# ducha-aiki/mods

Measured on AMD Instinct MI355X. Metric: image-pairs/sec (1024x768, HessAff+RootSIFT over the affine view ladder, MFMA FGINN match, LO-RANSAC H), higher is better.
Workload: dtype f32 (detect/describe) + u8 on the int8 matrix cores (distance matrix)

## Files before the change

### mods_amd/csrc/engine.hpp

```cpp
#pragma once
#include <hip/hip_runtime.h>
#include <stdint.h>
#include <stdlib.h>
#include <string.h>
#include <string>
#include <vector>
#include "../../include/modsx.h"
#include "kmath.hpp"

namespace mx {

#ifndef MODSX_MAXB
#define MODSX_MAXB 32
#endif
constexpr int MAXB = MODSX_MAXB;
constexpr int PAIR_GROUP = 4;
constexpr int NMS_MAXJ = 1024;
constexpr int MAX_TAPS = 17;

struct BlurJob {
  const float *src;
  float *blur;
  float *resp;
  int rows, cols;
// ... 8 lines not shown
  int tile0[MAXB + 1];
};
struct ResizeJob {
  const float *src;
  float *dst;
  float *resp;
  int srows, scols, drows, dcols;
  float norm;
  int pad;
};
struct ResizeBatch { ResizeJob j[MAXB]; int nj; int tile0[MAXB + 1]; };
struct NmsJob {
  const float *low, *cur, *high, *blur;
  int rows, cols, img, octave, level, pad;
};
struct NmsBatch {
  float posTh, negTh, finalTh;
  int border;
  double edgeScoreThreshold;
  int detType, pad;
};
struct Candidate {
  int img, octave, level, type;
  int r0, c0, r, c;
  float b0, b1, b2, val;
};

struct AffJob {
  const float *blur;
  int rows, cols;
  float x, y, s, pixelDistance;
};
struct AffOut { float u11, u12, u21, u22; int ok; int iters; };

struct OriJob {
  int img;
  float x, y, a11, a12, a21, a22;
};
constexpr int ORI_MAX_PEAKS = 18;

struct DescJob {
  int img;
  int P;
  int ksize;
  int tapOfs;
  float x, y, a11, a12, a21, a22;
  float i2p;
  int NC;
  int needOfs;
  int coordOfs;
  int touch;
  int outIdx;
  int rows0;
  int ro1;
  unsigned long long scratchOfs;
  unsigned long long rowOfs;
  unsigned long long gridOfs;
};
struct BlurTile {
  unsigned long long srcOfs, dstOfs;
  int P, NC, n, tapOfs, needOfs;
  int job, pad;
  int first, count, lo, span, magic;
};
struct ImgRef { const float *d; int rows, cols, pad; };
struct DescOut { float *f[MAXB]; uint8_t *u8[MAXB]; uint8_t *u8x[3][MAXB]; };

struct WarpJob {
  const float *src;
  float *dst;
  int srows, scols, drows, dcols;
  double M[6];
  float cval;
  int pad;
};

struct ViewJob {
  const float *src;
  float *rot, *tmp, *dst;
  int srows, scols, rrows, rcols, drows, dcols;
  int kx, ky, tapOfs, doBlur;
  int tileA, tileB;
  int tileF, fused;
  double R[6], W[6];
};

struct MatchRow {
  int t0, t1, nless, nbad;
  int tj;
  float dj;
  float d0, d1;
};
static_assert(sizeof(MatchRow) == 32, "match rows are 32 bytes");

struct DevBuf {
  void *p = nullptr;
  size_t cap = 0;
  bool ensure(size_t bytes);
  void release();
};
struct PinBuf {
  void *p = nullptr;
  size_t cap = 0;
  bool ensure(size_t bytes);
  void release();
};

struct Octave {
  int rows, cols;
  float pixelDistance;
  float *blur[8];
  float *resp[8];
};
struct Pyramid {
  int nOct = 0;
  Octave oct[24];
  DevBuf store;
};

void set_error(const std::string &s);
bool gpu_shared();
struct CtxBusy { modsx_ctx *c; explicit CtxBusy(modsx_ctx *c); ~CtxBusy(); CtxBusy(const CtxBusy &) = delete; CtxBusy &operator=(const CtxBusy &) = delete; };
hipError_t ctx_copy(modsx_ctx *c, void *dst, const void *src, size_t bytes, hipMemcpyKind kind);
hipError_t ctx_sync(modsx_ctx *c);
unsigned ctx_mark(modsx_ctx *c);
bool ctx_mark_reached(modsx_ctx *c, unsigned seq);
hipError_t ctx_wait_mark(modsx_ctx *c, unsigned seq);
bool host_wait_runtime();
int host_cpus_per_rank();
#define MX_HIP(expr)                                                                          \
  do {                                                                                        \
    hipError_t e_ = (expr);                                                                   \
    if (e_ != hipSuccess) {                                                                   \
      mx::set_error(std::string(#expr) + ": " + hipGetErrorString(e_));                       \
      return MODSX_ERR_DEVICE;                                                                \
    }                                                                                         \
  } while (0)

std::vector<float> gaussian_kernel(int n, double sigma);
int blur_ksize(float sigma);
void gauss_mask(float *mask, int size);
void circular_gauss_mask(float *mask, int size, float sigma);
const double *atan_lut_host();
inline bool check_borders_host(int w, int h, float ofsx, float ofsy, float a11, float a12, float a21, float a22, int rw, int rh) {
  return check_borders(w, h, ofsx, ofsy, a11, a12, a21, a22, rw, rh);
}
bool invert3(const double *S, double *t);
void rectify(double &a11, double &a12, double &a21, double &a22);

void launch_blur_hess(hipStream_t s, const BlurBatch &b, int nj, int maxRows, int maxCols);
void launch_hessian(hipStream_t s, const BlurBatch &b, int nj, int maxRows, int maxCols);
void launch_resize_half(hipStream_t s, const ResizeBatch &b, int nj, int maxRows, int maxCols);
void launch_nms(hipStream_t s, const NmsBatch &b, const NmsJob *jobs, const int *tilePrefix, const int *tileJob, int nj,
                int nTiles, int4 *queue, unsigned *qcount, unsigned qcap, Candidate *out, unsigned *counter, unsigned cap,
                const int *octFirst = nullptr, int levelsPerOctave = 0);
size_t cand_sort_temp_bytes(unsigned nsort);
int launch_cand_order(hipStream_t s, const Candidate *cand, const unsigned *counter, unsigned nsort, unsigned long long *keys,
                      unsigned long long *keys2, unsigned *idx, unsigned *idx2, void *temp, size_t tempBytes, unsigned long long *tabKey,
                      unsigned *tabRank, unsigned tabSize, unsigned *slotOf, Candidate *out, unsigned *outCount);
constexpr int NMS_QUEUES = 64;
constexpr int NMS_TILE_ROWS = 16;
void launch_gray(hipStream_t s, const void *src, float *dst, size_t n, int channels, int dtype);
void launch_baumberg(hipStream_t s, const AffJob *jobs, AffOut *out, int n, const float *mask, int W, int maxIter,
                     float convTh, float affInitialSigma);
constexpr int ATAN_CASES = 2048 + 64;
constexpr int ORI_NV = 1344;
void launch_orientation(hipStream_t s, const OriJob *jobs, float *out, int n, const ImgRef *imgs,
                        const unsigned short *maskIdx, const float *maskW,
                        const unsigned char *binTab, int doHalf, double th, int maxAngles);
void launch_trunc_u8(hipStream_t s, const float *src, uint8_t *dst, size_t n);
size_t mser_sort_blocks(const int *rows, int n);
void launch_mser_sort(hipStream_t s, const uint8_t *const *u8, const int *rows, const int *cols, const size_t *ordOfs, int n, int *blockHist,
                      int *start, int *order);
void launch_expand_blur_tiles(hipStream_t s, const DescJob *jobs, const int *prefixRows, const int *prefixCols, int nJobs,
                              const int *needTab, BlurTile *tilesRows, BlurTile *tilesCols, float2 *rowStarts);
void launch_sample_rows(hipStream_t s, const DescJob *jobs, const BlurTile *tiles, int nTiles, const ImgRef *imgs, const float *taps,
                        const int *needTab, float *dst, const float2 *rowStarts, float *dstGrid);
void launch_blur_cols(hipStream_t s, const BlurTile *tiles, int nTiles, const float *taps, const int *needTab, const float *src,
                      float *dst);
void launch_expand_tiles(hipStream_t s, const int *prefix, int nJobs, int *tileJob);
void launch_patch_sample(hipStream_t s, const DescJob *jobs, const int *tilePrefix, const int *tileJob, int nTiles,
                         const ImgRef *imgs, float *scratch);
void launch_patch_blur(hipStream_t s, const DescJob *jobs, const int *tilePrefix, const int *tileJob, int nTiles,
                       const float *taps, const int *needTab, const float *src, float *dst, int pass);
void launch_describe(hipStream_t s, const DescJob *jobs, int n, const ImgRef *imgs, const float *grid,
                     const int *needTab, const float *coordTab,
                     const float *mask, const unsigned short *maskIdx, int nmask, const float *oTab, const int *bins,
                     const double *wts, int photoNorm, int descTypes, int nOut, double maxBin, const DescOut &outs);
void launch_warp_affine(hipStream_t s, const WarpJob &jb);
void launch_blur_pass(hipStream_t s, const float *src, float *dst, int rows, int cols, const float *taps, int n, int pass, int border = 0);
void launch_sub(hipStream_t s, const float *a, const float *b, float *o, size_t n);
void launch_grad_products(hipStream_t s, const float *img, int rows, int cols, float *xx, float *yy, float *xy);
void launch_harris_combine(hipStream_t s, const float *bxx, const float *byy, const float *bxy, float sigmasq, float *o, size_t n);
void launch_views_warp(hipStream_t s, const ViewJob *jobs, int n, int tiles, int stage);
void launch_views_blur(hipStream_t s, const ViewJob *jobs, int n, int tiles, const float *taps, int pass);
constexpr int VF_TW = 128, VF_TH = 16, VF_RX = 32, VF_RY = 2;
void launch_views_rotblur(hipStream_t s, const ViewJob *jobs, int n, int tiles, const float *taps, int maxRx, int maxRy);
size_t match_workspace_bytes(int n1, int n2);
void launch_match(hipStream_t s, const uint8_t *d1, int n1, const uint8_t *d2, int n2, const double *pos2,
                  double sqminratio, double contrDistSq, int nn, MatchRow *rows, void *workspace);
#ifndef MODSX_SR_WIN
#define MODSX_SR_WIN 2400
#define MODSX_FC_ROWS 40
#define MODSX_SR_HALF 1
#define MODSX_SR_WGS 8
#endif
#ifndef MODSX_BLUR_LDS_C
#define MODSX_BLUR_LDS_C 9984
#endif
constexpr int MATCH_NN_MAX = 256;
constexpr int MATCH_MAXB = 4;
void launch_match_batch(hipStream_t s, int nb, const uint8_t *const *d1, const int *n1, const uint8_t *const *d2, const int *n2,
                        const double *const *pos2, double sqminratio, double contrDistSq, int nn, MatchRow *const *rows,
                        void *const *workspace, hipEvent_t *evSweep1 = nullptr);

}

namespace mx {
#ifdef MODSX_DUP_BUILD
int dup_count(int cls);
#define MX_DUP(cls) for (int dupLeft_ = mx::dup_count(cls); dupLeft_ > 0; dupLeft_--)
#else
#define MX_DUP(cls)
#endif
enum KClass { K_BLUR_HESS = 0, K_HESSIAN, K_RESIZE, K_NMS, K_BAUMBERG, K_ORIENT, K_PATCH_SAMPLE, K_BLUR_ROWS, K_DESCRIBE,
              K_MATCH, K_GRAY, K_WARP, K_VIEW_BLUR, K_BLUR_COLS, K_MATCH_SWEEP1, K_NCLASS };
struct Profiler {
  bool enabled = false;
  std::vector<hipEvent_t> evA, evB;
  std::vector<int> cls;
  size_t used = 0;
  double ms[K_NCLASS] = {0};
  double work[K_NCLASS] = {0};
  long launches[K_NCLASS] = {0};
};
}

struct modsx_image {
  float *d;
  int rows, cols;
  bool owned;
};

struct modsx_ctx {
  int dev;
  hipStream_t stream;
  mx::Pyramid pyr[mx::MAXB];
  mx::DevBuf candSort, candOut;
  size_t lastSurvivors = 0;
  mx::DevBuf nmsJobs, cand, counter, affJobs, affOut, oriJobs, oriOut, descJobs, tilePrefix, taps, imgRefs, scratchA, scratchB,
      descF[mx::MAXB], descU8[mx::MAXB], descAllF[2], descAllU8[2], descAllU8b[2], descCls[2][4][2], descU8x[3][mx::MAXB], shardLocal, pos2, matchRows, matchWork, misc, viewTmp[2], viewTaps, viewJobs, viewImg[mx::MAXB], scratchC, needTab, coordTab, tileJob, blurTiles, nmsQueue, rowStarts;
  mx::ImgRef imgRefsHost[mx::MAXB];
  mx::PinBuf hDescB;
  hipEvent_t descEv[2];
  bool descEvPending[2] = {false, false};
  bool descByEvent[2] = {true, true};
  unsigned descMark[2] = {0, 0};
  unsigned *hFlag = nullptr;
  unsigned flagSeq = 0;
  bool waitRuntime = true;
  mx::PinBuf hCand, hAff, hOri, hDesc, hMisc, hNms, hMatch, hViewTaps, hViewJobs, hMser, hRefs;
  float *dSmmMask = nullptr;
  int smmW = 0;
  std::vector<uint64_t> candKeys, candKeys2, candClaim;
  std::vector<uint32_t> candOrder, candOrder2;
  float *dOriMask = nullptr;
  unsigned short *dOriIdx = nullptr;
  float *dSiftMask = nullptr;
  unsigned short *dSiftMaskIdx = nullptr;
  int nSiftMask = 0;
  double *dAtan = nullptr;
  unsigned char *dOriBinTab = nullptr;
  float *dSiftOTab = nullptr;
  int *dSiftBins = nullptr;
  double *dSiftW = nullptr;
  double timings[6];
  mx::Profiler prof;
  size_t lastCandCount = 0;
  int busyDepth = 0;
  int shardLane = 0;
// ... 6 lines not shown
```

### mods_amd/csrc/engine_views.hip

```cpp
#include <math.h>
#include <algorithm>
#include <atomic>
#include <condition_variable>
#include <functional>
#include <mutex>
#include <thread>
#include "engine_api.hpp"

namespace mx {

int set_vs_pars(const double *scale_set, int ns, const double *tilt_set, int nt, double phi_base, double InitSigma,
                int doBlur, modsx_view *par, int cap, modsx_view *prev, int *nprev, int cap_prev) {
  const double eps1 = 0.01;
  std::vector<modsx_view> tmp;
  auto mk = [&](double phi, double tilt, double zoom, int blur) {
    modsx_view v; v.phi = phi; v.tilt = tilt; v.zoom = zoom; v.InitSigma = InitSigma; v.doBlur = blur;
    return v;
  };
  if (ns == 0 || nt == 0) tmp.push_back(mk(0, 0, 0, 0));
  for (int sc = 0; sc < ns; sc++)
    for (int t = 0; t < nt; t++) {
      if (fabs(tilt_set[t] - 1) > eps1) {
        int n_rot1 = floor(180.0 * tilt_set[t] / phi_base);
        double delta_phi = M_PI / n_rot1;
// ... 54 lines not shown
    P.ow = w; P.oh = h;
    return MODSX_OK;
  }
  P.identity = 0;
  double d, d2, w_new, h_new;
  double kV = 1., kH = 1.;
  if (zoomed) { kV = (double)w / (double)wS1; kH = (double)h / (double)hS1; }
  const bool q1 = (phi >= 0) && (phi < M_PI / 2);
  if (vertical_tilt) {
    if (q1) {
      w_new = floor((0.5 + cos(phi) * w + sin(phi) * h) / (kH));
      h_new = floor((0.5 + sin(phi) * w + cos(phi) * h) / (tilt * kV));
      H[0] = cos(phi) / kH; H[1] = sin(phi) / kH; H[2] = 0;
      H[3] = -sin(phi) / (tilt * kV); H[4] = cos(phi) / (tilt * kV); H[5] = floor(0.5 + sin(phi) * w / (tilt * kV));
    } else {
      w_new = floor((0.5 - cos(phi) * w + sin(phi) * h) / (kH));
      h_new = floor((0.5 + sin(phi) * w - cos(phi) * h) / (tilt * kV));
      d = -floor(cos(phi) * w / kH);
      d2 = floor(0.5 + (sin(phi) * w - cos(phi) * h) / (tilt * kV));
      H[0] = cos(phi) / kH; H[1] = sin(phi) / kH; H[2] = d;
      H[3] = -sin(phi) / (tilt * kV); H[4] = cos(phi) / (tilt * kV); H[5] = d2;
    }
  } else {
    if (q1) {
      w_new = floor((0.5 + cos(phi) * w + sin(phi) * h) / (tilt * kH));
      h_new = floor((0.5 + sin(phi) * w + cos(phi) * h) / (kV));
      H[0] = cos(phi) / (tilt * kH); H[1] = sin(phi) / (tilt * kH); H[2] = 0;
      H[3] = -sin(phi) / kV; H[4] = cos(phi) / kV; H[5] = floor(0.5 + sin(phi) * w / kV);
    } else {
      w_new = floor((0.5 - cos(phi) * w + sin(phi) * h) / (tilt * kH));
      h_new = floor((0.5 + sin(phi) * w - cos(phi) * h) / (kV));
      d = -floor(cos(phi) * w / (tilt * kH));
      d2 = floor(0.5 + (sin(phi) * w - cos(phi) * h) / kV);
      H[0] = cos(phi) / (tilt * kH); H[1] = sin(phi) / (tilt * kH); H[2] = d;
      H[3] = -sin(phi) / kV; H[4] = cos(phi) / kV; H[5] = d2;
    }
  }
  H[6] = 0; H[7] = 0; H[8] = 1;
  double sigma_aa_2 = zoomed ? InitSigma / (4.0 * zoom) : InitSigma / 2.0;
  double sigma_aa = InitSigma * tilt / (2.0 * zoom);
  double sigma_x = vertical_tilt ? sigma_aa_2 : sigma_aa, sigma_y = vertical_tilt ? sigma_aa : sigma_aa_2;
  double R[6];
  if (q1) {
    P.w_rot = floor((0.5 + cos(phi) * w + sin(phi) * h));
    P.h_rot = floor((0.5 + sin(phi) * w + cos(phi) * h));
    R[0] = cos(phi); R[1] = sin(phi); R[2] = 0;
    R[3] = -sin(phi); R[4] = cos(phi); R[5] = floor(0.5 + sin(phi) * w);
  } else {
    P.w_rot = floor((0.5 - cos(phi) * w + sin(phi) * h));
    P.h_rot = floor((0.5 + sin(phi) * w - cos(phi) * h));
    d = -floor(cos(phi) * w);
    d2 = floor(0.5 + (sin(phi) * w - cos(phi) * h));
    R[0] = cos(phi); R[1] = sin(phi); R[2] = d;
    R[3] = -sin(phi); R[4] = cos(phi); R[5] = d2;
  }
  P.ow = (int)w_new; P.oh = (int)h_new;
  if (P.w_rot <= 0 || P.h_rot <= 0 || P.ow <= 0 || P.oh <= 0) { set_error("degenerate synthesised view"); return MODSX_ERR_ARG; }
  invert_affine(R, P.Rinv);
  P.doBlur = v.doBlur;
  P.taps.clear();
  if (v.doBlur) {
    int kx = floor(2.0 * 3.0 * sigma_x + 1.0);
    if (kx % 2 == 0) kx++;
    if (kx < 3) kx = 3;
    int ky = floor(2.0 * 3.0 * sigma_y + 1.0);
    if (ky % 2 == 0) ky++;
    if (ky < 3) ky = 3;
    if (P.h_rot == 1) ky = 1;
    if (P.w_rot == 1) kx = 1;
    std::vector<float> KX = gaussian_kernel(kx, std::max(sigma_x, 0.));
    std::vector<float> KY = (ky == kx && fabs(sigma_x - sigma_y) < 2.220446049250313e-16) ? KX : gaussian_kernel(ky, std::max(sigma_y, 0.));
    P.kx = kx; P.ky = ky;
    P.taps = KX;
    P.taps.insert(P.taps.end(), KY.begin(), KY.end());
  }
  double Wz[6] = {0, 0, 0, 0, 0, 0};
  if (vertical_tilt) { Wz[0] = 1.0 / kH; Wz[4] = 1.0 / (tilt * kV); }
  else { Wz[0] = 1.0 / (tilt * kH); Wz[4] = 1.0 / kV; }
  invert_affine(Wz, P.Winv);
  return MODSX_OK;
}

static int synth_views_batch(modsx_ctx *c, const modsx_image *const *grays, const ViewPlan *P, float *const *dst, int n) {
  hipStream_t s = c->stream;
  std::vector<ViewJob> jobs;
  std::vector<float> taps;
  size_t rotFloats = 0;
  int tilesA = 0, tilesB = 0, tilesF = 0, maxRx = 0, maxRy = 0;
  double wpx = 0, rpx = 0;
  for (int i = 0; i < n; i++) {
    if (P[i].identity) continue;
    ViewJob j;
    memset(&j, 0, sizeof j);
    const modsx_image *gray = grays[i];
    j.src = gray->d; j.srows = gray->rows; j.scols = gray->cols;
    j.rrows = P[i].h_rot; j.rcols = P[i].w_rot; j.drows = P[i].oh; j.dcols = P[i].ow;
    j.dst = dst[i];
    j.doBlur = P[i].doBlur; j.kx = P[i].kx; j.ky = P[i].ky; j.tapOfs = (int)taps.size();
    taps.insert(taps.end(), P[i].taps.begin(), P[i].taps.end());
    for (int q = 0; q < 6; q++) { j.R[q] = P[i].Rinv[q]; j.W[q] = P[i].Winv[q]; }
    j.tileA = tilesA; j.tileB = tilesB; j.tileF = tilesF;
    j.fused = j.doBlur && (j.kx >> 1) <= VF_RX && (j.ky >> 1) <= VF_RY;
    if (j.fused) {
      tilesF += ((j.rcols + VF_TW - 1) / VF_TW) * ((j.rrows + VF_TH - 1) / VF_TH);
      maxRx = std::max(maxRx, j.kx >> 1); maxRy = std::max(maxRy, j.ky >> 1);
    } else
      tilesA += ((j.rcols + 63) / 64) * ((j.rrows + 3) / 4);
    tilesB += ((j.dcols + 63) / 64) * ((j.drows + 3) / 4);
    j.rot = (float *)(uintptr_t)rotFloats;
    rotFloats += (size_t)j.rrows * j.rcols;
    wpx += (double)gray->rows * gray->cols + 2.0 * j.rrows * j.rcols + (double)j.drows * j.dcols;
    rpx += (double)j.rrows * j.rcols;
    jobs.push_back(j);
  }
  if (jobs.empty()) return MODSX_OK;
  const size_t jobB = jobs.size() * sizeof(ViewJob), tapB = std::max<size_t>(1, taps.size()) * 4;
  if (!c->viewTmp[0].ensure(rotFloats * 4) || !c->viewTmp[1].ensure(rotFloats * 4) || !c->viewJobs.ensure(jobB + tapB + 64) ||
      !c->hViewJobs.ensure(jobB + tapB + 64))
    return MODSX_ERR_NOMEM;
  for (ViewJob &j : jobs) {
    const size_t o = (size_t)(uintptr_t)j.rot;
    j.rot = (float *)c->viewTmp[0].p + o;
    j.tmp = (float *)c->viewTmp[1].p + o;
  }
  char *hb = (char *)c->hViewJobs.p;
  memcpy(hb, jobs.data(), jobB);
  if (!taps.empty()) memcpy(hb + jobB, taps.data(), taps.size() * 4);
  MX_HIP(ctx_copy(c, c->viewJobs.p, hb, jobB + tapB, hipMemcpyHostToDevice));
  const ViewJob *dj = (const ViewJob *)c->viewJobs.p;
  const float *dt = (const float *)((char *)c->viewJobs.p + jobB);
  size_t pslot;
  prof_begin(c, K_WARP, wpx * 4, &pslot);
  launch_views_warp(s, dj, (int)jobs.size(), tilesA, 0);
  prof_end(c, pslot);
  prof_begin(c, K_VIEW_BLUR, rpx * 16, &pslot);
  launch_views_rotblur(s, dj, (int)jobs.size(), tilesF, dt, maxRx, maxRy);
  launch_views_blur(s, dj, (int)jobs.size(), tilesA, dt, 0);
  launch_views_blur(s, dj, (int)jobs.size(), tilesA, dt, 1);
  prof_end(c, pslot);
  prof_begin(c, K_WARP, 0, &pslot);
  launch_views_warp(s, dj, (int)jobs.size(), tilesB, 1);
  prof_end(c, pslot);
  MX_HIP(hipGetLastError());
  return MODSX_OK;
}

int synth_view(modsx_ctx *c, const modsx_image *gray, const modsx_view &v, modsx_image **out, double *H, int *identity, int) {
  *out = nullptr;
  ViewPlan P;
  int rc = plan_view(gray, v, P);
  if (rc) return rc;
  for (int i = 0; i < 9; i++) H[i] = P.H[i];
  *identity = P.identity;
  modsx_image *im = new modsx_image();
  im->rows = P.oh; im->cols = P.ow;
  if (P.identity) { im->d = gray->d; im->owned = false; *out = im; return MODSX_OK; }
  im->owned = true; im->d = nullptr;
  if (hipMalloc(&im->d, (size_t)P.ow * P.oh * 4) != hipSuccess) { delete im; set_error("hipMalloc view"); return MODSX_ERR_NOMEM; }
  float *dst[1] = {im->d};
  rc = synth_views_batch(c, &gray, &P, dst, 1);
  if (!rc && ctx_sync(c) != hipSuccess) { set_error("view synthesis failed"); rc = MODSX_ERR_DEVICE; }
  if (rc) { hipFree(im->d); delete im; return rc; }
  *out = im;
  return MODSX_OK;
}

int detect_describe_items(modsx_ctx *c, const modsx_image *const *itemImg, const int *itemView, int nitems, const modsx_view *views,
                          const modsx_pair_params &pp, std::vector<modsx_region> &regs,
                          float *devF, uint8_t *devU8, size_t devCapRegions, float *hostDesc, int *itemCounts,
                          const DescSet *dsIn, uint8_t *const *devU8x) {
  CtxBusy busy(c);
  regs.clear();
  DescSet ds;
  if (dsIn) ds = *dsIn;
  else { const int rd = resolve_descs(pp, nullptr, ds); if (rd) return rd; }
  const int oriHalf = ds.half() ? 1 : 0;
  if (!devU8x) { ds.forceHalf = oriHalf != 0; ds.n = 1; }
  if (itemCounts) for (int k = 0; k < nitems; k++) itemCounts[k] = 0;
  struct SetScope { SetScope() { host_set_enter(); } ~SetScope() { host_set_leave(); } } setScope;
  std::vector<int> take(nitems);
  for (int k = 0; k < nitems; k++) take[k] = k;
  size_t total = 0;
  for (size_t g0 = 0; g0 < take.size(); g0 += MAXB) {
    const int n = (int)std::min<size_t>(MAXB, take.size() - g0);
    modsx_image *vimg[MAXB];
    const modsx_image *cimg[MAXB];
    double Hs[MAXB][9], tilts[MAXB], zooms[MAXB];
    int ident[MAXB];
    int rc = MODSX_OK;
    for (int i = 0; i < n; i++) vimg[i] = nullptr;
    ViewPlan plans[MAXB];
    float *vdst[MAXB];
    const modsx_image *gimg[MAXB];
    for (int i = 0; i < n && !rc; i++) {
      const modsx_image *gray = itemImg[take[g0 + i]];
      gimg[i] = gray;
      const modsx_view &v = views[itemView[take[g0 + i]]];
      rc = plan_view(gray, v, plans[i]);
      if (rc) break;
      for (int q = 0; q < 9; q++) Hs[i][q] = plans[i].H[q];
      ident[i] = plans[i].identity;
      modsx_image *im = new modsx_image();
      im->rows = plans[i].oh; im->cols = plans[i].ow; im->owned = false;
      if (ident[i]) im->d = gray->d;
      else if (!c->viewImg[i].ensure((size_t)im->rows * im->cols * 4)) { delete im; rc = MODSX_ERR_NOMEM; break; }
      else im->d = (float *)c->viewImg[i].p;
      vdst[i] = im->d;
      vimg[i] = im;
      cimg[i] = im;
      tilts[i] = ident[i] ? 1.0 : fabs(v.tilt);
      zooms[i] = ident[i] ? 1.0 : v.zoom;
    }
    auto tnow = []() { return std::chrono::duration<double, std::milli>(std::chrono::steady_clock::now().time_since_epoch()).count(); };
    const bool tim = getenv("MODSX_HOST_TIMING") != nullptr;
    const bool tim2 = tim && atoi(getenv("MODSX_HOST_TIMING")) >= 2;
    double tq = 0;
    double t0 = tnow();
    if (!rc) rc = synth_views_batch(c, gimg, plans, vdst, n);
    if (tim) hipStreamSynchronize(c->stream);
    double t1 = tnow();
    std::vector<modsx_keypoint> kps[MAXB];
    std::vector<modsx_region> r0[MAXB], ro[MAXB];
    if (!rc) {
      if (pp.detector == MODSX_DET_MSER) {
        static const bool devSort = !(getenv("MODSX_MSER_DEVICE_SORT") && !atoi(getenv("MODSX_MSER_DEVICE_SORT")));
// ... 467 lines not shown
```

### mods_amd/csrc/kernels_views.hip

```cpp
#include "engine.hpp"

namespace mx {

MX_D void warp_xterm(const double *M, int x, int &adelta, int &bdelta) {
  const int AB_SCALE = 1024;
  adelta = (int)rint(M[0] * x * AB_SCALE); bdelta = (int)rint(M[3] * x * AB_SCALE);
}
MX_D void warp_yterm(const double *M, int y, int &X0, int &Y0) {
  const int AB_SCALE = 1024;
  X0 = (int)rint((M[1] * y + M[2]) * AB_SCALE) + 16;
  Y0 = (int)rint((M[4] * y + M[5]) * AB_SCALE) + 16;
}
MX_D float warp_fetch(const float *src, int sh, int sw, float cval, int adelta, int bdelta, int X0, int Y0) {
  const int X = (X0 + adelta) >> 5, Y = (Y0 + bdelta) >> 5;
  int sx = X >> 5, sy = Y >> 5;
  sx = sx < -32768 ? -32768 : (sx > 32767 ? 32767 : sx);
  sy = sy < -32768 ? -32768 : (sy > 32767 ? 32767 : sy);
  const float fx = (float)(X & 31) * (1.f / 32), fy = (float)(Y & 31) * (1.f / 32);
  const float w0 = (1.f - fy) * (1.f - fx), w1 = (1.f - fy) * fx, w2 = fy * (1.f - fx), w3 = fy * fx;
  float out;
  if (sx >= 0 && sx < sw - 1 && sy >= 0 && sy < sh - 1) {
    const float *S = src + (size_t)sy * sw + sx;
    out = S[0] * w0 + S[1] * w1 + S[sw] * w2 + S[sw + 1] * w3;
  } else if (sx >= sw || sx + 1 < 0 || sy >= sh || sy + 1 < 0) {
    out = cval;
  } else {
    const bool x0 = sx >= 0 && sx < sw, x1 = sx + 1 >= 0 && sx + 1 < sw, y0 = sy >= 0 && sy < sh, y1 = sy + 1 >= 0 && sy + 1 < sh;
    const float v0 = (x0 && y0) ? src[(size_t)sy * sw + sx] : cval;
    const float v1 = (x1 && y0) ? src[(size_t)sy * sw + sx + 1] : cval;
    const float v2 = (x0 && y1) ? src[(size_t)(sy + 1) * sw + sx] : cval;
    const float v3 = (x1 && y1) ? src[(size_t)(sy + 1) * sw + sx + 1] : cval;
    out = v0 * w0 + v1 * w1 + v2 * w2 + v3 * w3;
  }
  return out;
}
MX_D float warp_value(const float *src, int sh, int sw, const double *M, float cval, int x, int y) {
  int ad, bd, X0, Y0;
  warp_xterm(M, x, ad, bd);
  warp_yterm(M, y, X0, Y0);
  return warp_fetch(src, sh, sw, cval, ad, bd, X0, Y0);
}
MX_D void warp_body(const WarpJob &jb, int x, int y) {
  if (x >= jb.dcols || y >= jb.drows) return;
  jb.dst[(size_t)y * jb.dcols + x] = warp_value(jb.src, jb.srows, jb.scols, jb.M, jb.cval, x, y);
}
__global__ __launch_bounds__(256) void k_warp_affine(WarpJob jb) {
  warp_body(jb, blockIdx.x * 64 + (threadIdx.x & 63), blockIdx.y * 4 + (threadIdx.x >> 6));
}

MX_D int reflect101(int p, int n) {
  if (n == 1) return 0;
  while (p < 0 || p >= n) { if (p < 0) p = -p; else p = 2 * n - 2 - p; }
  return p;
}

MX_D int border_idx(int p, int n, int border) {
  if (border) return p < 0 ? 0 : (p > n - 1 ? n - 1 : p);
  return reflect101(p, n);
}
MX_D void blur_body(const float *src, float *dst, int rows, int cols, const float *taps, int n, int pass, int x, int y, int border = 0) {
  if (x >= cols || y >= rows) return;
  const int R = n >> 1;
  float v;
  if (n == 1) v = src[(size_t)y * cols + x];
  else if (pass == 0) {
    const float *row = src + (size_t)y * cols;
    if (n <= 5) {
      v = row[x] * taps[R];
      for (int j = 1; j <= R; j++) v = v + (row[border_idx(x - j, cols, border)] + row[border_idx(x + j, cols, border)]) * taps[R + j];
    } else {
      v = 0.f;
      for (int j = 0; j < n; j++) v = v + row[border_idx(x + j - R, cols, border)] * taps[j];
    }
  } else {
    v = taps[R] * src[(size_t)y * cols + x] + 0.f;
    for (int j = 1; j <= R; j++)
      v = v + taps[R + j] * (src[(size_t)border_idx(y + j, rows, border) * cols + x] + src[(size_t)border_idx(y - j, rows, border) * cols + x]);
  }
  dst[(size_t)y * cols + x] = v;
}
__global__ __launch_bounds__(256) void k_blur_pass(const float *src, float *dst, int rows, int cols, const float *taps,
                                                   int n, int pass, int border) {
  blur_body(src, dst, rows, cols, taps, n, pass, blockIdx.x * 64 + (threadIdx.x & 63), blockIdx.y * 4 + (threadIdx.x >> 6), border);
}

__global__ __launch_bounds__(256) void k_sub(const float *a, const float *b, float *o, size_t n) {
  const size_t i = (size_t)blockIdx.x * 256 + threadIdx.x;
  if (i < n) o[i] = a[i] - b[i];
}
__global__ __launch_bounds__(256) void k_grad_products(const float *img, int rows, int cols, float *xx, float *yy, float *xy) {
  const int c = blockIdx.x * 64 + (threadIdx.x & 63), r = blockIdx.y * 4 + (threadIdx.x >> 6);
  if (c >= cols || r >= rows) return;
  const float *R = img + (size_t)r * cols;
  float xg, yg;
  if (cols == 1) xg = 0.f;
  else if (c == 0) xg = R[c + 1] - R[c];
  else if (c == cols - 1) xg = R[c] - R[c - 1];
  else xg = R[c + 1] - R[c - 1];
  if (rows == 1) yg = 0.f;
  else if (r == 0) yg = R[cols + c] - R[c];
  else if (r == rows - 1) yg = R[c] - R[c - cols];
  else yg = R[cols + c] - R[c - cols];
  const size_t i = (size_t)r * cols + c;
  xx[i] = xg * xg; yy[i] = yg * yg; xy[i] = xg * yg;
}
__global__ __launch_bounds__(256) void k_harris_combine(const float *bxx, const float *byy, const float *bxy, float sigmasq, float *o, size_t n) {
  const size_t i = (size_t)blockIdx.x * 256 + threadIdx.x;
  if (i >= n) return;
  const float dx2 = bxx[i] * sigmasq, dy2 = byy[i] * sigmasq, dxdy = bxy[i] * sigmasq;
  const float s = dx2 + dy2;
  const float a = dx2 * dy2, b = dxdy * dxdy, c = (0.04f * s) * s;
  o[i] = (a - b) - c;
}

MX_D int find_view(const ViewJob *jobs, int n, int tile, int stage) {
  int j = 0;
  while (j + 1 < n && tile >= (stage == 2 ? jobs[j + 1].tileF : (stage ? jobs[j + 1].tileB : jobs[j + 1].tileA))) j++;
  return j;
}
__global__ __launch_bounds__(256) void k_views_warp(const ViewJob *jobs, int n, int stage) {
  const int j = find_view(jobs, n, blockIdx.x, stage);
  const ViewJob &v = jobs[j];
  WarpJob jb;
  if (stage == 0) { jb.src = v.src; jb.dst = v.rot; jb.srows = v.srows; jb.scols = v.scols; jb.drows = v.rrows; jb.dcols = v.rcols; }
  else { jb.src = v.rot; jb.dst = v.dst; jb.srows = v.rrows; jb.scols = v.rcols; jb.drows = v.drows; jb.dcols = v.dcols; }
#pragma unroll
  for (int i = 0; i < 6; i++) jb.M[i] = stage ? v.W[i] : v.R[i];
  jb.cval = 128.f;
  const int t = blockIdx.x - (stage ? v.tileB : v.tileA), tx = (jb.dcols + 63) / 64;
  warp_body(jb, (t % tx) * 64 + (threadIdx.x & 63), (t / tx) * 4 + (threadIdx.x >> 6));
}
__global__ __launch_bounds__(256) void k_views_blur(const ViewJob *jobs, int n, const float *taps, int pass) {
  const int j = find_view(jobs, n, blockIdx.x, 0);
  const ViewJob &v = jobs[j];
  if (!v.doBlur) return;
  const int t = blockIdx.x - v.tileA, tx = (v.rcols + 63) / 64;
  const float *src = pass ? v.tmp : v.rot;
  float *dst = pass ? v.rot : v.tmp;
  blur_body(src, dst, v.rrows, v.rcols, taps + v.tapOfs + (pass ? v.kx : 0), pass ? v.ky : v.kx, pass, (t % tx) * 64 + (threadIdx.x & 63),
            (t / tx) * 4 + (threadIdx.x >> 6));
}

template <int N>
MX_D void vf_rows(const float *Wt, float *Tt, const float *kxT, int WW, int Rx, int lane, int ty, int xOut, int yEnd, int nxRt) {
  constexpr int NK = N ? N : 1;
  float k[NK];
#pragma unroll
  for (int q = 0; q < NK; q++) k[q] = N ? kxT[q] : 0.f;
  for (int ly = ty; ly < yEnd; ly += 4) {
    const float *row = Wt + ly * WW + Rx;
    for (int lx = lane; lx < xOut; lx += 64) {
      float r;
      if (N == 1) r = row[lx];
      else if (N == 3 || N == 5) {
        constexpr int R = N >> 1;
        r = row[lx] * k[R];
#pragma unroll
        for (int q = 1; q <= R; q++) r = r + (row[lx - q] + row[lx + q]) * k[R + q];
      } else if (N > 5) {
        constexpr int R = N >> 1;
        r = 0.f;
#pragma unroll
        for (int q = 0; q < N; q++) r = r + row[lx + q - R] * k[q];
      } else {
        const int nx = nxRt;
        if (nx <= 5) {
          r = row[lx] * kxT[Rx];
          for (int q = 1; q <= Rx; q++) r = r + (row[lx - q] + row[lx + q]) * kxT[Rx + q];
        } else {
          r = 0.f;
          for (int q = 0; q < nx; q++) r = r + row[lx + q - Rx] * kxT[q];
        }
      }
      Tt[ly * VF_TW + lx] = r;
    }
  }
}
template <int N>
MX_D void vf_cols(const float *Tt, float *outBase, const float *kyT, int rcols, int Ry, int lane, int ty, int xOut, int yOut, int nyRt) {
  constexpr int NK = N ? N : 1;
  float k[NK];
#pragma unroll
  for (int q = 0; q < NK; q++) k[q] = N ? kyT[q] : 0.f;
  for (int ly = ty; ly < yOut; ly += 4) {
    const float *col = Tt + (ly + Ry) * VF_TW;
    float *out = outBase + (size_t)ly * rcols;
    for (int lx = lane; lx < xOut; lx += 64) {
      float r;
      if (N == 1) r = col[lx];
      else if (N > 1) {
        constexpr int R = N >> 1;
        r = k[R] * col[lx] + 0.f;
#pragma unroll
        for (int q = 1; q <= R; q++) r = r + k[R + q] * (col[lx + q * VF_TW] + col[lx - q * VF_TW]);
      } else {
        (void)nyRt;
        r = kyT[Ry] * col[lx] + 0.f;
        for (int q = 1; q <= Ry; q++) r = r + kyT[Ry + q] * (col[lx + q * VF_TW] + col[lx - q * VF_TW]);
      }
      out[lx] = r;
    }
  }
}

__global__ __launch_bounds__(256) void k_views_rotblur(const ViewJob *jobs, int n, const float *taps, int wFloats) {
  extern __shared__ float smem[];
  const int j = find_view(jobs, n, blockIdx.x, 2);
  const ViewJob &v = jobs[j];
  const int Rx = v.kx >> 1, Ry = v.ky >> 1;
  const int t = blockIdx.x - v.tileF, tx = (v.rcols + VF_TW - 1) / VF_TW;
  const int x0 = (t % tx) * VF_TW, y0 = (t / tx) * VF_TH;
  const int WW = VF_TW + 2 * Rx;
  float *const Wt = smem, *const Tt = smem + wFloats;
  const int lane = threadIdx.x & 63, ty = threadIdx.x >> 6;
  const int xEnd = min(VF_TW, v.rcols - x0) + 2 * Rx, yEnd = min(VF_TH, v.rrows - y0) + 2 * Ry;
  {
    constexpr int NX = (VF_TW + 2 * VF_RX + 63) / 64;
    int ad[NX], bd[NX];
#pragma unroll
    for (int u = 0; u < NX; u++) warp_xterm(v.R, reflect101(x0 - Rx + lane + 64 * u, v.rcols), ad[u], bd[u]);
    for (int ly = ty; ly < yEnd; ly += 4) {
      int X0, Y0;
      warp_yterm(v.R, reflect101(y0 - Ry + ly, v.rrows), X0, Y0);
#pragma unroll
      for (int u = 0; u < NX; u++) {
        const int lx = lane + 64 * u;
        if (lx < xEnd) Wt[ly * WW + lx] = warp_fetch(v.src, v.srows, v.scols, 128.f, ad[u], bd[u], X0, Y0);
      }
    }
  }
  __syncthreads();
  const float *kxT = taps + v.tapOfs, *kyT = kxT + v.kx;
  const int nx = v.kx, ny = v.ky, xOut = xEnd - 2 * Rx, yOut = yEnd - 2 * Ry;
  switch (nx) {
    case 1: vf_rows<1>(Wt, Tt, kxT, WW, Rx, lane, ty, xOut, yEnd, nx); break;
    case 3: vf_rows<3>(Wt, Tt, kxT, WW, Rx, lane, ty, xOut, yEnd, nx); break;
    case 5: vf_rows<5>(Wt, Tt, kxT, WW, Rx, lane, ty, xOut, yEnd, nx); break;
    case 7: vf_rows<7>(Wt, Tt, kxT, WW, Rx, lane, ty, xOut, yEnd, nx); break;
    case 9: vf_rows<9>(Wt, Tt, kxT, WW, Rx, lane, ty, xOut, yEnd, nx); break;
    case 11: vf_rows<11>(Wt, Tt, kxT, WW, Rx, lane, ty, xOut, yEnd, nx); break;
    case 13: vf_rows<13>(Wt, Tt, kxT, WW, Rx, lane, ty, xOut, yEnd, nx); break;
    default: vf_rows<0>(Wt, Tt, kxT, WW, Rx, lane, ty, xOut, yEnd, nx); break;
  }
  __syncthreads();
  float *const outBase = v.rot + (size_t)y0 * v.rcols + x0;
  switch (ny) {
    case 1: vf_cols<1>(Tt, outBase, kyT, v.rcols, Ry, lane, ty, xOut, yOut, ny); break;
    case 3: vf_cols<3>(Tt, outBase, kyT, v.rcols, Ry, lane, ty, xOut, yOut, ny); break;
    case 5: vf_cols<5>(Tt, outBase, kyT, v.rcols, Ry, lane, ty, xOut, yOut, ny); break;
    default: vf_cols<0>(Tt, outBase, kyT, v.rcols, Ry, lane, ty, xOut, yOut, ny); break;
  }
}

void launch_warp_affine(hipStream_t s, const WarpJob &jb) {
  dim3 grid((jb.dcols + 63) / 64, (jb.drows + 3) / 4);
  hipLaunchKernelGGL(k_warp_affine, grid, dim3(256), 0, s, jb);
}
void launch_blur_pass(hipStream_t s, const float *src, float *dst, int rows, int cols, const float *taps, int n, int pass, int border) {
  dim3 grid((cols + 63) / 64, (rows + 3) / 4);
  hipLaunchKernelGGL(k_blur_pass, grid, dim3(256), 0, s, src, dst, rows, cols, taps, n, pass, border);
}
void launch_sub(hipStream_t s, const float *a, const float *b, float *o, size_t n) {
  hipLaunchKernelGGL(k_sub, dim3((unsigned)((n + 255) / 256)), dim3(256), 0, s, a, b, o, n);
}
void launch_grad_products(hipStream_t s, const float *img, int rows, int cols, float *xx, float *yy, float *xy) {
  hipLaunchKernelGGL(k_grad_products, dim3((cols + 63) / 64, (rows + 3) / 4), dim3(256), 0, s, img, rows, cols, xx, yy, xy);
}
void launch_harris_combine(hipStream_t s, const float *bxx, const float *byy, const float *bxy, float sigmasq, float *o, size_t n) {
  hipLaunchKernelGGL(k_harris_combine, dim3((unsigned)((n + 255) / 256)), dim3(256), 0, s, bxx, byy, bxy, sigmasq, o, n);
}
void launch_views_warp(hipStream_t s, const ViewJob *jobs, int n, int tiles, int stage) {
  if (tiles > 0) MX_DUP(K_WARP) hipLaunchKernelGGL(k_views_warp, dim3(tiles), dim3(256), 0, s, jobs, n, stage);
}
void launch_views_blur(hipStream_t s, const ViewJob *jobs, int n, int tiles, const float *taps, int pass) {
  if (tiles > 0) hipLaunchKernelGGL(k_views_blur, dim3(tiles), dim3(256), 0, s, jobs, n, taps, pass);
}
void launch_views_rotblur(hipStream_t s, const ViewJob *jobs, int n, int tiles, const float *taps, int maxRx, int maxRy) {
  if (tiles <= 0) return;
  const int wFloats = (VF_TH + 2 * maxRy) * (VF_TW + 2 * maxRx), tFloats = (VF_TH + 2 * maxRy) * VF_TW;
  MX_DUP(K_VIEW_BLUR) hipLaunchKernelGGL(k_views_rotblur, dim3(tiles), dim3(256), (size_t)(wFloats + tFloats) * 4, s, jobs, n, taps, wFloats);
}

}
```

Baseline: 215.5.

## Fuse rotate, blur and axis-aligned tilt warp into one tiled view kernel

```diff
diff --git a/mods_amd/csrc/engine.hpp b/mods_amd/csrc/engine.hpp
--- a/mods_amd/csrc/engine.hpp
+++ b/mods_amd/csrc/engine.hpp
@@ -114,7 +114,9 @@
   int kx, ky, tapOfs, doBlur;
   int tileA, tileB;
   int tileF, fused;
+  int tileG, pad;
   double R[6], W[6];
+  double invW[2];
 };
 
 struct MatchRow {
@@ -228,6 +230,7 @@
 void launch_views_blur(hipStream_t s, const ViewJob *jobs, int n, int tiles, const float *taps, int pass);
 constexpr int VF_TW = 128, VF_TH = 16, VF_RX = 32, VF_RY = 2;
 void launch_views_rotblur(hipStream_t s, const ViewJob *jobs, int n, int tiles, const float *taps, int maxRx, int maxRy);
+void launch_views_fused(hipStream_t s, const ViewJob *jobs, int n, int tiles, const float *taps, int maxRx, int maxRy);
 size_t match_workspace_bytes(int n1, int n2);
 void launch_match(hipStream_t s, const uint8_t *d1, int n1, const uint8_t *d2, int n2, const double *pos2,
                   double sqminratio, double contrDistSq, int nn, MatchRow *rows, void *workspace);
diff --git a/mods_amd/csrc/engine_views.hip b/mods_amd/csrc/engine_views.hip
--- a/mods_amd/csrc/engine_views.hip
+++ b/mods_amd/csrc/engine_views.hip
@@ -160,12 +160,13 @@
 }
 
 static int synth_views_batch(modsx_ctx *c, const modsx_image *const *grays, const ViewPlan *P, float *const *dst, int n) {
+  static const bool separate = getenv("MODSX_VIEWS_SEPARATE") && atoi(getenv("MODSX_VIEWS_SEPARATE"));
   hipStream_t s = c->stream;
   std::vector<ViewJob> jobs;
   std::vector<float> taps;
-  size_t rotFloats = 0;
-  int tilesA = 0, tilesB = 0, tilesF = 0, maxRx = 0, maxRy = 0;
-  double wpx = 0, rpx = 0;
+  size_t rotFloats = 0, tmpFloats = 0;
+  int tilesA = 0, tilesB = 0, tilesF = 0, tilesG = 0, maxRx = 0, maxRy = 0, maxRxG = 0, maxRyG = 0;
+  double pxRot = 0, pxBlur = 0, pxFused = 0, pxTilt = 0;
   for (int i = 0; i < n; i++) {
     if (P[i].identity) continue;
     ViewJob j;
@@ -177,29 +178,44 @@
     j.doBlur = P[i].doBlur; j.kx = P[i].kx; j.ky = P[i].ky; j.tapOfs = (int)taps.size();
     taps.insert(taps.end(), P[i].taps.begin(), P[i].taps.end());
     for (int q = 0; q < 6; q++) { j.R[q] = P[i].Rinv[q]; j.W[q] = P[i].Winv[q]; }
-    j.tileA = tilesA; j.tileB = tilesB; j.tileF = tilesF;
+    j.tileA = tilesA; j.tileB = tilesB; j.tileF = tilesF; j.tileG = tilesG;
+    const double srcPx = (double)gray->rows * gray->cols, rotPx = (double)j.rrows * j.rcols, dstPx = (double)j.drows * j.dcols;
     j.fused = j.doBlur && (j.kx >> 1) <= VF_RX && (j.ky >> 1) <= VF_RY;
-    if (j.fused) {
-      tilesF += ((j.rcols + VF_TW - 1) / VF_TW) * ((j.rrows + VF_TH - 1) / VF_TH);
-      maxRx = std::max(maxRx, j.kx >> 1); maxRy = std::max(maxRy, j.ky >> 1);
-    } else
-      tilesA += ((j.rcols + 63) / 64) * ((j.rrows + 3) / 4);
-    tilesB += ((j.dcols + 63) / 64) * ((j.drows + 3) / 4);
-    j.rot = (float *)(uintptr_t)rotFloats;
-    rotFloats += (size_t)j.rrows * j.rcols;
-    wpx += (double)gray->rows * gray->cols + 2.0 * j.rrows * j.rcols + (double)j.drows * j.dcols;
-    rpx += (double)j.rrows * j.rcols;
+    if (j.fused && !separate && j.W[1] == 0 && j.W[3] == 0 && j.W[0] > 0 && j.W[4] > 0) j.fused = 2;
+    const int tilesV = ((j.rcols + VF_TW - 1) / VF_TW) * ((j.rrows + VF_TH - 1) / VF_TH);
+    if (j.fused == 2) {
+      tilesG += tilesV;
+      maxRxG = std::max(maxRxG, j.kx >> 1); maxRyG = std::max(maxRyG, j.ky >> 1);
+      j.invW[0] = 1.0 / j.W[0]; j.invW[1] = 1.0 / j.W[4];
+      pxFused += srcPx + dstPx;
+    } else {
+      if (j.fused) {
+        tilesF += tilesV;
+        maxRx = std::max(maxRx, j.kx >> 1); maxRy = std::max(maxRy, j.ky >> 1);
+        pxBlur += srcPx + rotPx;
+      } else {
+        tilesA += ((j.rcols + 63) / 64) * ((j.rrows + 3) / 4);
+        pxRot += srcPx + rotPx;
+        if (j.doBlur) pxBlur += 4 * rotPx;
+        j.tmp = (float *)(uintptr_t)tmpFloats;
+        tmpFloats += (size_t)j.rrows * j.rcols;
+      }
+      tilesB += ((j.dcols + 63) / 64) * ((j.drows + 3) / 4);
+      pxTilt += rotPx + dstPx;
+      j.rot = (float *)(uintptr_t)rotFloats;
+      rotFloats += (size_t)j.rrows * j.rcols;
+    }
     jobs.push_back(j);
   }
   if (jobs.empty()) return MODSX_OK;
   const size_t jobB = jobs.size() * sizeof(ViewJob), tapB = std::max<size_t>(1, taps.size()) * 4;
-  if (!c->viewTmp[0].ensure(rotFloats * 4) || !c->viewTmp[1].ensure(rotFloats * 4) || !c->viewJobs.ensure(jobB + tapB + 64) ||
+  if (!c->viewTmp[0].ensure(rotFloats * 4) || !c->viewTmp[1].ensure(tmpFloats * 4) || !c->viewJobs.ensure(jobB + tapB + 64) ||
       !c->hViewJobs.ensure(jobB + tapB + 64))
     return MODSX_ERR_NOMEM;
   for (ViewJob &j : jobs) {
-    const size_t o = (size_t)(uintptr_t)j.rot;
-    j.rot = (float *)c->viewTmp[0].p + o;
-    j.tmp = (float *)c->viewTmp[1].p + o;
+    if (j.fused == 2) continue;
+    j.rot = (float *)c->viewTmp[0].p + (size_t)(uintptr_t)j.rot;
+    j.tmp = j.fused ? nullptr : (float *)c->viewTmp[1].p + (size_t)(uintptr_t)j.tmp;
   }
   char *hb = (char *)c->hViewJobs.p;
   memcpy(hb, jobs.data(), jobB);
@@ -207,18 +223,30 @@
   MX_HIP(ctx_copy(c, c->viewJobs.p, hb, jobB + tapB, hipMemcpyHostToDevice));
   const ViewJob *dj = (const ViewJob *)c->viewJobs.p;
   const float *dt = (const float *)((char *)c->viewJobs.p + jobB);
+  const int nj = (int)jobs.size();
   size_t pslot;
-  prof_begin(c, K_WARP, wpx * 4, &pslot);
-  launch_views_warp(s, dj, (int)jobs.size(), tilesA, 0);
-  prof_end(c, pslot);
-  prof_begin(c, K_VIEW_BLUR, rpx * 16, &pslot);
-  launch_views_rotblur(s, dj, (int)jobs.size(), tilesF, dt, maxRx, maxRy);
-  launch_views_blur(s, dj, (int)jobs.size(), tilesA, dt, 0);
-  launch_views_blur(s, dj, (int)jobs.size(), tilesA, dt, 1);
-  prof_end(c, pslot);
-  prof_begin(c, K_WARP, 0, &pslot);
-  launch_views_warp(s, dj, (int)jobs.size(), tilesB, 1);
-  prof_end(c, pslot);
+  if (tilesG > 0) {
+    prof_begin(c, K_VIEW_BLUR, pxFused * 4, &pslot);
+    launch_views_fused(s, dj, nj, tilesG, dt, maxRxG, maxRyG);
+    prof_end(c, pslot);
+  }
+  if (tilesA > 0) {
+    prof_begin(c, K_WARP, pxRot * 4, &pslot);
+    launch_views_warp(s, dj, nj, tilesA, 0);
+    prof_end(c, pslot);
+  }
+  if (tilesF > 0 || tilesA > 0) {
+    prof_begin(c, K_VIEW_BLUR, pxBlur * 4, &pslot);
+    launch_views_rotblur(s, dj, nj, tilesF, dt, maxRx, maxRy);
+    launch_views_blur(s, dj, nj, tilesA, dt, 0);
+    launch_views_blur(s, dj, nj, tilesA, dt, 1);
+    prof_end(c, pslot);
+  }
+  if (tilesB > 0) {
+    prof_begin(c, K_WARP, pxTilt * 4, &pslot);
+    launch_views_warp(s, dj, nj, tilesB, 1);
+    prof_end(c, pslot);
+  }
   MX_HIP(hipGetLastError());
   return MODSX_OK;
 }
diff --git a/mods_amd/csrc/kernels_views.hip b/mods_amd/csrc/kernels_views.hip
--- a/mods_amd/csrc/kernels_views.hip
+++ b/mods_amd/csrc/kernels_views.hip
@@ -21,7 +21,10 @@
   float out;
   if (sx >= 0 && sx < sw - 1 && sy >= 0 && sy < sh - 1) {
     const float *S = src + (size_t)sy * sw + sx;
-    out = S[0] * w0 + S[1] * w1 + S[sw] * w2 + S[sw + 1] * w3;
+    float2 a, b;
+    __builtin_memcpy(&a, S, 8);
+    __builtin_memcpy(&b, S + sw, 8);
+    out = a.x * w0 + a.y * w1 + b.x * w2 + b.y * w3;
   } else if (sx >= sw || sx + 1 < 0 || sy >= sh || sy + 1 < 0) {
     out = cval;
   } else {
@@ -114,9 +117,14 @@
 }
 
 MX_D int find_view(const ViewJob *jobs, int n, int tile, int stage) {
-  int j = 0;
-  while (j + 1 < n && tile >= (stage == 2 ? jobs[j + 1].tileF : (stage ? jobs[j + 1].tileB : jobs[j + 1].tileA))) j++;
-  return j;
+  int lo = 0, hi = n - 1;
+  while (lo < hi) {
+    const int mid = (lo + hi + 1) >> 1;
+    const ViewJob &m = jobs[mid];
+    const int first = stage == 3 ? m.tileG : (stage == 2 ? m.tileF : (stage ? m.tileB : m.tileA));
+    if (tile >= first) lo = mid; else hi = mid - 1;
+  }
+  return lo;
 }
 __global__ __launch_bounds__(256) void k_views_warp(const ViewJob *jobs, int n, int stage) {
   const int j = find_view(jobs, n, blockIdx.x, stage);
@@ -142,6 +150,47 @@
 }
 
 template <int N>
+MX_D float vf_row_value(const float *row, int lx, const float *k, const float *kxT, int Rx, int nx) {
+  float r;
+  if (N == 1) r = row[lx];
+  else if (N == 3 || N == 5) {
+    constexpr int R = N >> 1;
+    r = row[lx] * k[R];
+#pragma unroll
+    for (int q = 1; q <= R; q++) r = r + (row[lx - q] + row[lx + q]) * k[R + q];
+  } else if (N > 5) {
+    constexpr int R = N >> 1;
+    r = 0.f;
+#pragma unroll
+    for (int q = 0; q < N; q++) r = r + row[lx + q - R] * k[q];
+  } else {
+    if (nx <= 5) {
+      r = row[lx] * kxT[Rx];
+      for (int q = 1; q <= Rx; q++) r = r + (row[lx - q] + row[lx + q]) * kxT[Rx + q];
+    } else {
+      r = 0.f;
+      for (int q = 0; q < nx; q++) r = r + row[lx + q - Rx] * kxT[q];
+    }
+  }
+  return r;
+}
+template <int N>
+MX_D float vf_col_value(const float *col, int lx, int stride, const float *k, const float *kyT, int Ry) {
+  float r;
+  if (N == 1) r = col[lx];
+  else if (N > 1) {
+    constexpr int R = N >> 1;
+    r = k[R] * col[lx] + 0.f;
+#pragma unroll
+    for (int q = 1; q <= R; q++) r = r + k[R + q] * (col[lx + q * stride] + col[lx - q * stride]);
+  } else {
+    r = kyT[Ry] * col[lx] + 0.f;
+    for (int q = 1; q <= Ry; q++) r = r + kyT[Ry + q] * (col[lx + q * stride] + col[lx - q * stride]);
+  }
+  return r;
+}
+
+template <int N>
 MX_D void vf_rows(const float *Wt, float *Tt, const float *kxT, int WW, int Rx, int lane, int ty, int xOut, int yEnd, int nxRt) {
   constexpr int NK = N ? N : 1;
   float k[NK];
@@ -149,31 +198,7 @@
   for (int q = 0; q < NK; q++) k[q] = N ? kxT[q] : 0.f;
   for (int ly = ty; ly < yEnd; ly += 4) {
     const float *row = Wt + ly * WW + Rx;
-    for (int lx = lane; lx < xOut; lx += 64) {
-      float r;
-      if (N == 1) r = row[lx];
-      else if (N == 3 || N == 5) {
-        constexpr int R = N >> 1;
-        r = row[lx] * k[R];
-#pragma unroll
-        for (int q = 1; q <= R; q++) r = r + (row[lx - q] + row[lx + q]) * k[R + q];
-      } else if (N > 5) {
-        constexpr int R = N >> 1;
-        r = 0.f;
-#pragma unroll
-        for (int q = 0; q < N; q++) r = r + row[lx + q - R] * k[q];
-      } else {
-        const int nx = nxRt;
-        if (nx <= 5) {
-          r = row[lx] * kxT[Rx];
-          for (int q = 1; q <= Rx; q++) r = r + (row[lx - q] + row[lx + q]) * kxT[Rx + q];
-        } else {
-          r = 0.f;
-          for (int q = 0; q < nx; q++) r = r + row[lx + q - Rx] * kxT[q];
-        }
-      }
-      Tt[ly * VF_TW + lx] = r;
-    }
+    for (int lx = lane; lx < xOut; lx += 64) Tt[ly * VF_TW + lx] = vf_row_value<N>(row, lx, k, kxT, Rx, nxRt);
   }
 }
 template <int N>
@@ -182,24 +207,11 @@
   float k[NK];
 #pragma unroll
   for (int q = 0; q < NK; q++) k[q] = N ? kyT[q] : 0.f;
+  (void)nyRt;
   for (int ly = ty; ly < yOut; ly += 4) {
     const float *col = Tt + (ly + Ry) * VF_TW;
     float *out = outBase + (size_t)ly * rcols;
-    for (int lx = lane; lx < xOut; lx += 64) {
-      float r;
-      if (N == 1) r = col[lx];
-      else if (N > 1) {
-        constexpr int R = N >> 1;
-        r = k[R] * col[lx] + 0.f;
-#pragma unroll
-        for (int q = 1; q <= R; q++) r = r + k[R + q] * (col[lx + q * VF_TW] + col[lx - q * VF_TW]);
-      } else {
-        (void)nyRt;
-        r = kyT[Ry] * col[lx] + 0.f;
-        for (int q = 1; q <= Ry; q++) r = r + kyT[Ry + q] * (col[lx + q * VF_TW] + col[lx - q * VF_TW]);
-      }
-      out[lx] = r;
-    }
+    for (int lx = lane; lx < xOut; lx += 64) out[lx] = vf_col_value<N>(col, lx, VF_TW, k, kyT, Ry);
   }
 }
 
@@ -252,6 +264,152 @@
   }
 }
 
+constexpr int VG_TS = VF_TW + 1;
+constexpr int VG_HR = VF_TH + 2 * VF_RY + 1;
+constexpr int VG_TABS = VF_TW + 4 + VF_TH + 4;
+
+MX_D int warp_tap0(const double *M, int axis, int p) {
+  int ad, bd, X0, Y0;
+  warp_xterm(M, axis ? 0 : p, ad, bd);
+  warp_yterm(M, axis ? p : 0, X0, Y0);
+  const int s = ((axis ? Y0 + bd : X0 + ad) >> 5) >> 5;
+  return s < -32768 ? -32768 : (s > 32767 ? 32767 : s);
+}
+MX_D int first_reaching(const double *M, int axis, int target, int n, int lim, double inv) {
+  if (target <= 0) return 0;
+  if (target >= lim) return n;
+  const double h = ((double)target - M[axis ? 5 : 2]) * inv;
+  int p = h > 0. ? (h < (double)n ? (int)h : n) : 0;
+  while (p > 0 && warp_tap0(M, axis, p - 1) >= target) p--;
+  while (p < n && warp_tap0(M, axis, p) < target) p++;
+  return p;
+}
+MX_D float warp_fetch_tile(const float *Bt, int WW, int x0, int y0, int sh, int sw, float cval, int adelta, int bdelta, int X0, int Y0) {
+  const int X = (X0 + adelta) >> 5, Y = (Y0 + bdelta) >> 5;
+  int sx = X >> 5, sy = Y >> 5;
+  sx = sx < -32768 ? -32768 : (sx > 32767 ? 32767 : sx);
+  sy = sy < -32768 ? -32768 : (sy > 32767 ? 32767 : sy);
+  const float fx = (float)(X & 31) * (1.f / 32), fy = (float)(Y & 31) * (1.f / 32);
+  const float w0 = (1.f - fy) * (1.f - fx), w1 = (1.f - fy) * fx, w2 = fy * (1.f - fx), w3 = fy * fx;
+  float out;
+  if (sx >= 0 && sx < sw - 1 && sy >= 0 && sy < sh - 1) {
+    const float *S = Bt + (sy - y0) * WW + (sx - x0);
+    out = S[0] * w0 + S[1] * w1 + S[WW] * w2 + S[WW + 1] * w3;
+  } else if (sx >= sw || sx + 1 < 0 || sy >= sh || sy + 1 < 0) {
+    out = cval;
+  } else {
+    const bool bx0 = sx >= 0 && sx < sw, bx1 = sx + 1 >= 0 && sx + 1 < sw, by0 = sy >= 0 && sy < sh, by1 = sy + 1 >= 0 && sy + 1 < sh;
+    const float v0 = (bx0 && by0) ? Bt[(sy - y0) * WW + (sx - x0)] : cval;
+    const float v1 = (bx1 && by0) ? Bt[(sy - y0) * WW + (sx + 1 - x0)] : cval;
+    const float v2 = (bx0 && by1) ? Bt[(sy + 1 - y0) * WW + (sx - x0)] : cval;
+    const float v3 = (bx1 && by1) ? Bt[(sy + 1 - y0) * WW + (sx + 1 - x0)] : cval;
+    out = v0 * w0 + v1 * w1 + v2 * w2 + v3 * w3;
+  }
+  return out;
+}
+struct FlatWalk {
+  int o, i, dq, dr, n;
+  MX_D FlatWalk(int tid, int inner) : o(tid / inner), i(tid - (tid / inner) * inner), dq(256 / inner), dr(256 - (256 / inner) * inner), n(inner) {}
+  MX_D void next() { o += dq; i += dr; if (i >= n) { i -= n; o++; } }
+};
+template <int N>
+MX_D void vg_rows(const float *Wt, float *Tt, const unsigned char *colTab, const float *kxT, int WW, int Rx, int tid, int nix, int yEnd, int nxRt) {
+  constexpr int NK = N ? N : 1;
+  float k[NK];
+#pragma unroll
+  for (int q = 0; q < NK; q++) k[q] = N ? kxT[q] : 0.f;
+  for (FlatWalk w(tid, nix); w.o < yEnd; w.next()) {
+    const int lc = colTab[w.i];
+    if (lc != 255) Tt[w.o * VG_TS + lc] = vf_row_value<N>(Wt + w.o * WW + Rx, lc, k, kxT, Rx, nxRt);
+  }
+}
+template <int N>
+MX_D void vg_cols(const float *Tt, float *Bt, const unsigned char *colTab, const unsigned char *rowTab, const float *kyT, int WW, int Ry, int tid,
+                  int nix, int niy) {
+  constexpr int NK = N ? N : 1;
+  float k[NK];
+#pragma unroll
+  for (int q = 0; q < NK; q++) k[q] = N ? kyT[q] : 0.f;
+  for (FlatWalk w(tid, nix); w.o < niy; w.next()) {
+    const int lc = colTab[w.i], lr = rowTab[w.o];
+    if (lc != 255 && lr != 255) Bt[lr * WW + lc] = vf_col_value<N>(Tt + (lr + Ry) * VG_TS, lc, VG_TS, k, kyT, Ry);
+  }
+}
+__global__ __launch_bounds__(256) void k_views_fused(const ViewJob *jobs, int n, const float *taps, int wFloats, int tFloats) {
+  extern __shared__ float smem[];
+  const int j = find_view(jobs, n, blockIdx.x, 3);
+  const ViewJob &v = jobs[j];
+  const int Rx = v.kx >> 1, Ry = v.ky >> 1;
+  const int t = blockIdx.x - v.tileG, tx = (v.rcols + VF_TW - 1) / VF_TW;
+  const int x0 = (t % tx) * VF_TW, y0 = (t / tx) * VF_TH;
+  const int x1 = min(x0 + VF_TW, v.rcols), y1 = min(y0 + VF_TH, v.rrows);
+  __shared__ int own[4];
+  {
+    const int axis = threadIdx.x >> 7, upper = (threadIdx.x >> 6) & 1;
+    const int r = first_reaching(v.W, axis, axis ? (upper ? y1 : y0) : (upper ? x1 : x0), axis ? v.drows : v.dcols, axis ? v.rrows : v.rcols, v.invW[axis]);
+    if ((threadIdx.x & 63) == 0) own[threadIdx.x >> 6] = r;
+  }
+  __syncthreads();
+  const int xa = own[0], xb = own[1], ya = own[2], yb = own[3];
+  const int nox = xb - xa, noy = yb - ya;
+  if (nox <= 0 || noy <= 0) return;
+  const int colsB = x1 - x0 + (x1 < v.rcols ? 1 : 0), rowsB = y1 - y0 + (y1 < v.rrows ? 1 : 0);
+  const int xEnd = colsB + 2 * Rx, yEnd = rowsB + 2 * Ry;
+  const int WW = VF_TW + 2 * Rx + 1;
+  float *const Wt = smem, *const Tt = smem + wFloats;
+  unsigned char *const colTab = (unsigned char *)(smem + wFloats + tFloats), *const rowTab = colTab + VF_TW + 4;
+  const int tid = threadIdx.x;
+  const bool denseX = 2 * nox >= colsB, denseY = 2 * noy >= rowsB;
+  const int nix = denseX ? colsB : 2 * nox, niy = denseY ? rowsB : 2 * noy;
+  {
+    int *const colAd = (int *)Tt, *const colBd = colAd + WW, *const rowX0 = colBd + WW, *const rowY0 = rowX0 + VG_HR;
+    for (int i = tid; i < xEnd + yEnd; i += 256) {
+      if (i < xEnd) warp_xterm(v.R, reflect101(x0 - Rx + i, v.rcols), colAd[i], colBd[i]);
+      else warp_yterm(v.R, reflect101(y0 - Ry + i - xEnd, v.rrows), rowX0[i - xEnd], rowY0[i - xEnd]);
+    }
+    for (int i = tid; i < nix + niy; i += 256) {
+      if (i < nix) {
+        const int lc = denseX ? i : warp_tap0(v.W, 0, xa + (i >> 1)) + (i & 1) - x0;
+        colTab[i] = (unsigned char)(lc >= 0 && lc < colsB ? lc : 255);
+      } else {
+        const int q = i - nix, lr = denseY ? q : warp_tap0(v.W, 1, ya + (q >> 1)) + (q & 1) - y0;
+        rowTab[q] = (unsigned char)(lr >= 0 && lr < rowsB ? lr : 255);
+      }
+    }
+    __syncthreads();
+    for (FlatWalk w(tid, xEnd); w.o < yEnd; w.next())
+      Wt[w.o * WW + w.i] = warp_fetch(v.src, v.srows, v.scols, 128.f, colAd[w.i], colBd[w.i], rowX0[w.o], rowY0[w.o]);
+  }
+  __syncthreads();
+  const float *kxT = taps + v.tapOfs, *kyT = kxT + v.kx;
+  const int nx = v.kx, ny = v.ky;
+  switch (nx) {
+    case 1: vg_rows<1>(Wt, Tt, colTab, kxT, WW, Rx, tid, nix, yEnd, nx); break;
+    case 3: vg_rows<3>(Wt, Tt, colTab, kxT, WW, Rx, tid, nix, yEnd, nx); break;
+    case 5: vg_rows<5>(Wt, Tt, colTab, kxT, WW, Rx, tid, nix, yEnd, nx); break;
+    case 7: vg_rows<7>(Wt, Tt, colTab, kxT, WW, Rx, tid, nix, yEnd, nx); break;
+    case 9: vg_rows<9>(Wt, Tt, colTab, kxT, WW, Rx, tid, nix, yEnd, nx); break;
+    case 11: vg_rows<11>(Wt, Tt, colTab, kxT, WW, Rx, tid, nix, yEnd, nx); break;
+    case 13: vg_rows<13>(Wt, Tt, colTab, kxT, WW, Rx, tid, nix, yEnd, nx); break;
+    default: vg_rows<0>(Wt, Tt, colTab, kxT, WW, Rx, tid, nix, yEnd, nx); break;
+  }
+  __syncthreads();
+  switch (ny) {
+    case 1: vg_cols<1>(Tt, Wt, colTab, rowTab, kyT, WW, Ry, tid, nix, niy); break;
+    case 3: vg_cols<3>(Tt, Wt, colTab, rowTab, kyT, WW, Ry, tid, nix, niy); break;
+    case 5: vg_cols<5>(Tt, Wt, colTab, rowTab, kyT, WW, Ry, tid, nix, niy); break;
+    default: vg_cols<0>(Tt, Wt, colTab, rowTab, kyT, WW, Ry, tid, nix, niy); break;
+  }
+  __syncthreads();
+  for (FlatWalk w(tid, nox); w.o < noy; w.next()) {
+    const int x = xa + w.i, y = ya + w.o;
+    int ad, bd, X0, Y0;
+    warp_xterm(v.W, x, ad, bd);
+    warp_yterm(v.W, y, X0, Y0);
+    v.dst[(size_t)y * v.dcols + x] = warp_fetch_tile(Wt, WW, x0, y0, v.rrows, v.rcols, 128.f, ad, bd, X0, Y0);
+  }
+}
+
 void launch_warp_affine(hipStream_t s, const WarpJob &jb) {
   dim3 grid((jb.dcols + 63) / 64, (jb.drows + 3) / 4);
   hipLaunchKernelGGL(k_warp_affine, grid, dim3(256), 0, s, jb);
@@ -280,5 +438,13 @@
   const int wFloats = (VF_TH + 2 * maxRy) * (VF_TW + 2 * maxRx), tFloats = (VF_TH + 2 * maxRy) * VF_TW;
   MX_DUP(K_VIEW_BLUR) hipLaunchKernelGGL(k_views_rotblur, dim3(tiles), dim3(256), (size_t)(wFloats + tFloats) * 4, s, jobs, n, taps, wFloats);
 }
-
-}
+void launch_views_fused(hipStream_t s, const ViewJob *jobs, int n, int tiles, const float *taps, int maxRx, int maxRy) {
+  if (tiles <= 0) return;
+  const int wFloats = (VF_TH + 2 * maxRy + 1) * (VF_TW + 2 * maxRx + 1), tFloats = (VF_TH + 2 * maxRy + 1) * VG_TS;
+  static_assert(2 * (VF_TW + 2 * VF_RX + 1) + 2 * VG_HR <= (VF_TH + 1) * VG_TS, "the rotation's column / row terms fit the row-filtered tile");
+  static_assert(VF_TW + 1 < 255 && VF_TH + 1 < 255, "tapped columns / rows are listed as bytes");
+  MX_DUP(K_VIEW_BLUR) hipLaunchKernelGGL(k_views_fused, dim3(tiles), dim3(256), (size_t)(wFloats + tFloats) * 4 + ((VG_TABS + 3) & ~3), s, jobs, n, taps,
+                                         wFloats, tFloats);
+}
+
+}
```

Result: faster. 217.7 (median of 6 runs) (+1.0%).
